# preethamam/AutomaticPanoramicImageStitching-AutoPanoStitch-MATLAB

Hardware: NVIDIA B200
Metric: descriptor_pairs_per_sec (higher is better)
Workload: dtype f16

## Files before the change

### automaticpanoramicimagestitching-autopanostitch-matlab_b200/csrc/aps_knn_tc.cu

```cuda
#include "aps_tc_ptx.cuh"

#pragma nv_diag_suppress 128

namespace {
using namespace aps_tc;

constexpr int TM = 128;
constexpr int RB = 2;
constexpr int TN = 128;
constexpr int NUM_B_STAGES = 4;
constexpr int NUM_ACC_SLOTS = 2 * RB;
constexpr int NUM_CS_STAGES = 8;
constexpr int KC = 8;
constexpr int CSPLIT = 1;
constexpr int MAX_SEG = 4 / CSPLIT;
constexpr int NUM_EPI_WARPS = 4 * RB * CSPLIT;
constexpr int FIRST_EPI_WARP = 1 + RB;
constexpr int NUM_THREADS = 32 * (FIRST_EPI_WARP + NUM_EPI_WARPS);
static_assert(NUM_ACC_SLOTS * TN == 512, "TMEM budget");

struct Barriers {
  uint64_t b_full[NUM_B_STAGES], b_empty[NUM_B_STAGES];
  uint64_t a_full, a_empty;
  uint64_t acc_full[NUM_ACC_SLOTS], acc_empty[NUM_ACC_SLOTS];
  uint64_t cs_full[NUM_CS_STAGES], cs_empty[NUM_CS_STAGES];
  uint32_t tmem_base;
  uint32_t pad;
};

__device__ __forceinline__ float4 lds_f32x4(uint32_t a) {
  float4 v;
  asm volatile("ld.shared.v4.f32 {%0, %1, %2, %3}, [%4];" : "=f"(v.x), "=f"(v.y), "=f"(v.z), "=f"(v.w) : "r"(a));
  return v;
}
__device__ __forceinline__ uint32_t lds_u32(uint32_t a) { uint32_t v; asm volatile("ld.shared.u32 %0, [%1];" : "=r"(v) : "r"(a)); return v; }
__device__ __forceinline__ void sts_u32(uint32_t a, uint32_t v) { asm volatile("st.shared.u32 [%0], %1;" ::"r"(a), "r"(v) : "memory"); }
constexpr uint32_t SLOT_STRIDE = TM * 4;

struct KParams {
  int64_t q0, q1, t0, t1;
  int dp;
  int nslot;
  int units_full;
  int tail_units;
  int tail_seg;
  int64_t tile_lo;
  int64_t tile_hi;
  int tiles_per_seg;
  int tail_balanced;
  int grid;
  const float* colscale;
// ... 69 lines not shown
__device__ __forceinline__ void top2_of_32(float (&v)[32]) {
#pragma unroll
  for (int i = 0; i < 32; i += 2) {
    const float a = v[i], b = v[i + 1];
    v[i] = fmaxf(a, b);
    v[i + 1] = fminf(a, b);
  }
#pragma unroll
  for (int st = 2; st < 32; st *= 2)
#pragma unroll
    for (int i = 0; i < 32; i += 2 * st) top2_merge(v[i], v[i + 1], v[i + st], v[i + st + 1]);
}
__device__ __forceinline__ void insert3(float x, uint32_t px, float& l1, float& l2, float& l3, uint32_t& p1, uint32_t& p2,
                                        uint32_t& p3) {
  const bool c1 = x > l1, c2 = x > l2, c3 = x > l3;
  l3 = c2 ? l2 : (c3 ? x : l3);
  p3 = c2 ? p2 : (c3 ? px : p3);
  l2 = c1 ? l1 : (c2 ? x : l2);
  p2 = c1 ? p1 : (c2 ? px : p2);
  l1 = c1 ? x : l1;
  p1 = c1 ? px : p1;
}
constexpr uint32_t kKeyFloorBits = 0xff7fff80u;
constexpr int threads_for(int cs) { return 32 * (1 + RB + 4 * RB * cs); }

template <bool BIAS, bool DUMP, bool PRE, int KCT, int CS = CSPLIT>
__global__ void __launch_bounds__(threads_for(CS), 1)
k_knn_tc(const __grid_constant__ CUtensorMap map_q, const __grid_constant__ CUtensorMap map_t, const KParams Pin) {
  if (Pin.variant_flag && ((*Pin.variant_flag != 0) != (Pin.variant_want != 0))) return;
  extern __shared__ __align__(1024) uint8_t smem_raw[];
  uint8_t* smem = (uint8_t*)(((uintptr_t)smem_raw + 1023) & ~(uintptr_t)1023);
  const int a_bytes = TM * Pin.dp * 2, b_bytes = TN * Pin.dp * 2;
  uint8_t* smem_a = smem;
  uint8_t* smem_b = smem_a + RB * a_bytes;
  float* smem_cs = (float*)(smem_b + NUM_B_STAGES * b_bytes);
  uint32_t* smem_topi = (uint32_t*)(smem_cs + NUM_CS_STAGES * 2 * TN);
  Barriers* bars = (Barriers*)(smem_topi + RB * CS * KC * TM);

  const int warp = threadIdx.x >> 5, lane = threadIdx.x & 31;
  const int ksl = Pin.dp / KSLAB;
  const int kst = Pin.dp / 16;
  KParams P = Pin;
  if (P.nrows_dev) {
    const int64_t n = *P.nrows_dev;
    P.q1 = P.q0 + n;
    P.units_full = 0;
    P.tail_units = (int)((n + RB * TM - 1) / (RB * TM));
  }
  const int64_t num_units = P.unit_table ? P.n_table_units
                            : (P.tail_balanced ? (int64_t)P.units_full + (int64_t)P.tail_balanced * P.grid
                                               : (int64_t)P.units_full + (int64_t)P.tail_units * P.tail_seg);

  if (threadIdx.x == 0) {
    for (int i = 0; i < NUM_B_STAGES; ++i) { mbar_init(&bars->b_full[i], 1); mbar_init(&bars->b_empty[i], RB); }
    mbar_init(&bars->a_full, 1);
    mbar_init(&bars->a_empty, RB);
    for (int i = 0; i < NUM_ACC_SLOTS; ++i) { mbar_init(&bars->acc_full[i], 1); mbar_init(&bars->acc_empty[i], 4 * CS); }
    for (int i = 0; i < NUM_CS_STAGES; ++i) { mbar_init(&bars->cs_full[i], 1); mbar_init(&bars->cs_empty[i], (4 * RB * CS)); }
    asm volatile("fence.mbarrier_init.release.cluster;" ::: "memory");
  }
  if (warp == 1) {
    asm volatile("tcgen05.alloc.cta_group::1.sync.aligned.shared::cta.b32 [%0], %1;" ::"r"(smem_u32(&bars->tmem_base)), "r"(512) : "memory");
    asm volatile("tcgen05.relinquish_alloc_permit.cta_group::1.sync.aligned;" ::: "memory");
  }
  tc_fence_before();
  __syncthreads();
  tc_fence_after();
  const uint32_t tmem_base = bars->tmem_base;

  if (warp == 0) {
    if (elect_one()) {
      uint32_t bs = 0, bph = 0, aph = 0, cs = 0, cph = 0;
      for (int64_t u = blockIdx.x; u < num_units; u += gridDim.x) {
        const Unit x = get_unit(P, u);
        if (x.tl >= x.th) continue;
        mbar_wait_backoff(&bars->a_empty, aph ^ 1);
        mbar_arrive_expect_tx(&bars->a_full, (uint32_t)(RB * a_bytes));
        for (int r = 0; r < RB; ++r)
          for (int s = 0; s < ksl; ++s)
            tma_load_2d(smem_a + r * a_bytes + s * (TM * 128), &map_q, s * KSLAB,
                        (int)(x.qrow0 + r * TM), &bars->a_full);
        aph ^= 1;
        for (int64_t t = x.tl; t < x.th; ++t) {
          mbar_wait_backoff(&bars->cs_empty[cs], cph ^ 1);
          mbar_arrive_expect_tx(&bars->cs_full[cs], (BIAS ? 2u : 1u) * TN * (uint32_t)sizeof(float));
          bulk_load_1d(smem_cs + cs * 2 * TN, P.colscale + t * TN, TN * (uint32_t)sizeof(float), &bars->cs_full[cs]);
          if (BIAS)
            bulk_load_1d(smem_cs + cs * 2 * TN + TN, P.colbias + t * TN, TN * (uint32_t)sizeof(float), &bars->cs_full[cs]);
          if (++cs == NUM_CS_STAGES) { cs = 0; cph ^= 1; }
          mbar_wait_backoff(&bars->b_empty[bs], bph ^ 1);
          mbar_arrive_expect_tx(&bars->b_full[bs], (uint32_t)b_bytes);
          for (int s = 0; s < ksl; ++s)
            tma_load_2d(smem_b + bs * b_bytes + s * (TN * 128), &map_t, s * KSLAB, (int)(t * TN), &bars->b_full[bs]);
          if (++bs == NUM_B_STAGES) { bs = 0; bph ^= 1; }
        }
      }
    }
  } else if (warp <= RB) {
    if (elect_one()) {
      const int r = warp - 1;
      const uint32_t idesc = P.idesc;
      const uint32_t a_addr = smem_u32(smem_a + r * a_bytes);
      uint32_t bs = 0, bph = 0, aph = 0, tcount = 0;
      for (int64_t u = blockIdx.x; u < num_units; u += gridDim.x) {
        const Unit x = get_unit(P, u);
        if (x.tl >= x.th) continue;
        mbar_wait(&bars->a_full, aph);
        aph ^= 1;
        for (int64_t t = x.tl; t < x.th; ++t, ++tcount) {
          const uint32_t slot = (tcount & 1) * RB + r, acph = (tcount >> 1) & 1;
          mbar_wait(&bars->acc_empty[slot], acph ^ 1);
          mbar_wait(&bars->b_full[bs], bph);
          tc_fence_after();
          const uint32_t b_addr = smem_u32(smem_b + bs * b_bytes);
          const uint32_t d_tmem = tmem_base + slot * TN;
          for (int k = 0; k < kst; ++k) {
            const int slab = k >> 2, kin = k & 3;
            const uint64_t adesc = make_kmajor_sw128_desc(a_addr + slab * (TM * 128) + kin * 32);
            const uint64_t bdesc = make_kmajor_sw128_desc(b_addr + slab * (TN * 128) + kin * 32);
            umma_bf16(d_tmem, adesc, bdesc, idesc, k > 0 ? 1u : 0u);
          }
          tc_commit(&bars->acc_full[slot]);
          tc_commit(&bars->b_empty[bs]);
          if (++bs == NUM_B_STAGES) { bs = 0; bph ^= 1; }
        }
        tc_commit(&bars->a_empty);
      }
    }
  } else {
    const int quad = warp & 3;
    const int egrp = (warp - FIRST_EPI_WARP) >> 2;
    const int grp = egrp / CS;
    const int ch = egrp % CS;
    constexpr int CG = TN / CS;
    const int row_in_tile = quad * 32 + lane;
    const uint32_t si = smem_u32(smem_topi + (egrp * KC) * TM + row_in_tile);
    uint32_t tcount = 0;
    for (int64_t u = blockIdx.x; u < num_units; u += gridDim.x) {
      const Unit x = get_unit(P, u);
      if (x.skip) continue;
      const int64_t qrow = x.qrow0 + grp * TM + row_in_tile;
      if constexpr (KCT == 3) {
        float l1 = __uint_as_float(kKeyFloorBits), l2 = l1, l3 = l1;
        uint32_t p1 = 0xffffffffu, p2 = 0xffffffffu, p3 = 0xffffffffu;
        for (int64_t t = x.tl; t < x.th; ++t, ++tcount) {
          const uint32_t slot = (tcount & 1) * RB + grp, acph = (tcount >> 1) & 1;
          const uint32_t cs = tcount % NUM_CS_STAGES, cph = (tcount / NUM_CS_STAGES) & 1;
          mbar_wait(&bars->acc_full[slot], acph);
          mbar_wait(&bars->cs_full[cs], cph);
          tc_fence_after();
          const uint32_t cscale = smem_u32(smem_cs + cs * 2 * TN + ch * CG);
          const int64_t col0 = t * TN + ch * CG;
          const bool partial = (col0 < x.t0) || (col0 + CG > x.t1);
          const uint32_t taddr = tmem_base + ((uint32_t)(quad * 32) << 16) + slot * TN + ch * CG;
          float m1 = __uint_as_float(kKeyFloorBits), m2 = m1;
#pragma unroll 1
          for (int c = 0; c < CG / 32; ++c) {
            float cur[32];
            tmem_ld32(taddr + c * 32, cur);
            tmem_wait_ld(cur);
#pragma unroll
            for (int g = 0; g < 4; ++g) {
              const float4 s0 = lds_f32x4(cscale + (c * 32 + 8 * g) * 4);
              const float4 s1 = lds_f32x4(cscale + (c * 32 + 8 * g + 4) * 4);
              if (BIAS) {
                const float4 b0 = lds_f32x4(cscale + (TN + c * 32 + 8 * g) * 4);
                const float4 b1 = lds_f32x4(cscale + (TN + c * 32 + 8 * g + 4) * 4);
                cur[8 * g + 0] = fmaf(cur[8 * g + 0], s0.x, b0.x); cur[8 * g + 1] = fmaf(cur[8 * g + 1], s0.y, b0.y);
                cur[8 * g + 2] = fmaf(cur[8 * g + 2], s0.z, b0.z); cur[8 * g + 3] = fmaf(cur[8 * g + 3], s0.w, b0.w);
                cur[8 * g + 4] = fmaf(cur[8 * g + 4], s1.x, b1.x); cur[8 * g + 5] = fmaf(cur[8 * g + 5], s1.y, b1.y);
                cur[8 * g + 6] = fmaf(cur[8 * g + 6], s1.z, b1.z); cur[8 * g + 7] = fmaf(cur[8 * g + 7], s1.w, b1.w);
              } else {
                cur[8 * g + 0] *= s0.x; cur[8 * g + 1] *= s0.y; cur[8 * g + 2] *= s0.z; cur[8 * g + 3] *= s0.w;
                cur[8 * g + 4] *= s1.x; cur[8 * g + 5] *= s1.y; cur[8 * g + 6] *= s1.z; cur[8 * g + 7] *= s1.w;
              }
            }
            const uint32_t cbase = (uint32_t)(ch * CG + c * 32);
#pragma unroll
            for (int j = 0; j < 32; ++j)
              cur[j] = __uint_as_float((__float_as_uint(cur[j]) & ~127u) | (cbase + (uint32_t)j));
            if (partial) {
              const int lo = (int)max(x.t0 - col0, (int64_t)0) - c * 32, hi = (int)min(x.t1 - col0, (int64_t)CG) - c * 32;
#pragma unroll
              for (int j = 0; j < 32; ++j)
                if (j < lo || j >= hi) cur[j] = __uint_as_float(kKeyFloorBits | (cbase + (uint32_t)j));
            }
            top2_of_32(cur);
            top2_merge(m1, m2, cur[0], cur[1]);
          }
          tc_fence_before();
          __syncwarp();
          if (lane == 0) {
            mbar_arrive(&bars->acc_empty[slot]);
            mbar_arrive(&bars->cs_empty[cs]);
          }
          const uint32_t base = (uint32_t)(t * TN);
          insert3(m1, base + (__float_as_uint(m1) & 127u), l1, l2, l3, p1, p2, p3);
          insert3(m2, base + (__float_as_uint(m2) & 127u), l1, l2, l3, p1, p2, p3);
        }
        if (qrow < x.qend) {
          const int64_t o = (x.out_row + grp * TM + row_in_tile) * P.cand_stride + ch * 3;
          const float floor_v = -1.0e38f;
          P.cand_idx[o + 0] = l1 > floor_v ? p1 : 0xffffffffu; P.cand_score[o + 0] = l1 > floor_v ? l1 : -CUDART_INF_F;
          P.cand_idx[o + 1] = l2 > floor_v ? p2 : 0xffffffffu; P.cand_score[o + 1] = l2 > floor_v ? l2 : -CUDART_INF_F;
          P.cand_idx[o + 2] = l3 > floor_v ? p3 : 0xffffffffu; P.cand_score[o + 2] = l3 > floor_v ? l3 : -CUDART_INF_F;
        }
        continue;
      }
      float bv[KCT];
#pragma unroll
      for (int i = 0; i < KCT; ++i) {
        bv[i] = __uint_as_float(0xff7ffff8u | (uint32_t)i);
        sts_u32(si + i * SLOT_STRIDE, 0xffffffffu);
      }
      float theta = bv[KCT - 1];
      int minpos = KCT - 1;
      float4 tb_next = (PRE && x.tl < x.th) ? __ldg(P.tile_bounds + x.tl) : make_float4(0.f, 0.f, 0.f, 0.f);
      for (int64_t t = x.tl; t < x.th; ++t, ++tcount) {
        const uint32_t slot = (tcount & 1) * RB + grp, acph = (tcount >> 1) & 1;
        const uint32_t cs = tcount % NUM_CS_STAGES, cph = (tcount / NUM_CS_STAGES) & 1;
        mbar_wait(&bars->acc_full[slot], acph);
        mbar_wait(&bars->cs_full[cs], cph);
        tc_fence_after();
        const uint32_t cscale = smem_u32(smem_cs + cs * 2 * TN + ch * CG);
        const int64_t col0 = t * TN + ch * CG;
        const bool partial = (col0 < x.t0) || (col0 + CG > x.t1);
        const uint32_t taddr = tmem_base + ((uint32_t)(quad * 32) << 16) + slot * TN + ch * CG;
        const float4 tb = tb_next;
        if (PRE && t + 1 < x.th) tb_next = __ldg(P.tile_bounds + t + 1);
        auto pre_threshold = [&](float th) {
          const float num = th - tb.z - 1.0e-6f * (fabsf(th) + fabsf(tb.z));
          return num * (num >= 0.f ? tb.x : tb.y);
        };
        float thr_pre = PRE ? pre_threshold(theta) : 0.f;
        float va[32], vb[32];
        bool slot_released = false;
        if constexpr (PRE && CS == 1 && !DUMP) {
#ifndef APS_TC_NOEPI
          float rm[16];
          tmem_ld32(taddr, va);
          tmem_wait_ld(va);
#pragma unroll
          for (int c = 0; c < 4; ++c) {
            float(&cur)[32] = (c & 1) ? vb : va;
            float(&nxt)[32] = (c & 1) ? va : vb;
            if (c + 1 < 4) tmem_ld32(taddr + (c + 1) * 32, nxt);
#pragma unroll
            for (int g = 0; g < 4; ++g) {
              float m = fmaxf(fmaxf(cur[8 * g], cur[8 * g + 1]), cur[8 * g + 2]);
              m = fmaxf(fmaxf(m, cur[8 * g + 3]), cur[8 * g + 4]);
              m = fmaxf(fmaxf(m, cur[8 * g + 5]), cur[8 * g + 6]);
              rm[4 * c + g] = fmaxf(m, cur[8 * g + 7]);
            }
            if (c + 1 < 4) tmem_wait_ld(nxt);
          }
          float tmax = fmaxf(fmaxf(rm[0], rm[1]), rm[2]);
#pragma unroll
          for (int g = 3; g < 15; g += 2) tmax = fmaxf(fmaxf(tmax, rm[g]), rm[g + 1]);
          tmax = fmaxf(tmax, rm[15]);
          if (__any_sync(0xffffffffu, partial || tmax > thr_pre)) {
            uint32_t pend = 0;
#pragma unroll
            for (int g = 0; g < 16; ++g) pend |= (rm[g] > thr_pre) ? (1u << g) : 0u;
            if (partial) pend = 0xffffu;
            uint32_t uni = __reduce_or_sync(0xffffffffu, pend);
            auto search_group = [&](float(&v)[8], const int g) {
              const float4 s0 = lds_f32x4(cscale + (8 * g) * 4);
              const float4 s1 = lds_f32x4(cscale + (8 * g + 4) * 4);
              if (BIAS) {
                const float4 b0 = lds_f32x4(cscale + (TN + 8 * g) * 4);
                const float4 b1 = lds_f32x4(cscale + (TN + 8 * g + 4) * 4);
                v[0] = fmaf(v[0], s0.x, b0.x); v[1] = fmaf(v[1], s0.y, b0.y);
                v[2] = fmaf(v[2], s0.z, b0.z); v[3] = fmaf(v[3], s0.w, b0.w);
                v[4] = fmaf(v[4], s1.x, b1.x); v[5] = fmaf(v[5], s1.y, b1.y);
                v[6] = fmaf(v[6], s1.z, b1.z); v[7] = fmaf(v[7], s1.w, b1.w);
              } else {
                v[0] *= s0.x; v[1] *= s0.y; v[2] *= s0.z; v[3] *= s0.w;
                v[4] *= s1.x; v[5] *= s1.y; v[6] *= s1.z; v[7] *= s1.w;
              }
              if (partial) {
#pragma unroll
                for (int j = 0; j < 8; ++j) {
                  const int64_t col = col0 + 8 * g + j;
                  if (col < x.t0 || col >= x.t1) v[j] = -CUDART_INF_F;
                }
              }
              float gm = fmaxf(fmaxf(v[0], v[1]), v[2]);
              gm = fmaxf(fmaxf(gm, v[3]), v[4]);
              gm = fmaxf(fmaxf(gm, v[5]), v[6]);
              gm = fmaxf(gm, v[7]);
              while (gm > theta) {
                int js = 7;
#pragma unroll
                for (int j = 6; j >= 0; --j) js = (v[j] == gm) ? j : js;
                sts_u32(si + minpos * SLOT_STRIDE, (uint32_t)(col0 + 8 * g + js));
                const float key = __uint_as_float((__float_as_uint(gm) & ~7u) | (uint32_t)minpos);
#pragma unroll
                for (int i = 0; i < KCT; ++i) bv[i] = (i == minpos) ? key : bv[i];
                if constexpr (KCT == 8) {
                  float m01 = fminf(fminf(bv[0], bv[1]), bv[2]);
                  float m23 = fminf(fminf(bv[3], bv[4]), bv[5]);
                  theta = fminf(fminf(m01, m23), fminf(bv[6], bv[7]));
                } else if constexpr (KCT == 6) {
                  theta = fminf(fminf(fminf(bv[0], bv[1]), bv[2]), fminf(fminf(bv[3], bv[4]), bv[5]));
                } else {
                  theta = fminf(fminf(bv[0], bv[1]), fminf(bv[2], bv[3]));
                }
                minpos = (int)(__float_as_uint(theta) & 7u);
#pragma unroll
                for (int j = 0; j < 8; ++j) v[j] = (j == js) ? -CUDART_INF_F : v[j];
                gm = fmaxf(fmaxf(v[0], v[1]), v[2]);
                gm = fmaxf(fmaxf(gm, v[3]), v[4]);
                gm = fmaxf(fmaxf(gm, v[5]), v[6]);
                gm = fmaxf(gm, v[7]);
              }
            };
            while (uni) {
              int gq[4];
#pragma unroll
              for (int q = 0; q < 4; ++q) {
                gq[q] = uni ? __ffs((int)uni) - 1 : 31;
                uni &= uni - 1;
              }
              float vs[32];
              __syncwarp();
#pragma unroll
              for (int q = 0; q < 4; ++q) tmem_ld8(taddr + 8 * (gq[q] & 15), *reinterpret_cast<float(*)[8]>(vs + 8 * q));
              tmem_wait_ld(vs);
              if (uni == 0u) {
                tc_fence_before();
                __syncwarp();
                if (lane == 0) mbar_arrive(&bars->acc_empty[slot]);
                slot_released = true;
              }
#pragma unroll
              for (int q = 0; q < 4; ++q)
                if ((pend >> gq[q]) & 1u) search_group(*reinterpret_cast<float(*)[8]>(vs + 8 * q), gq[q]);
            }
          }
#endif
        } else {
        if (CS == 1) {
          tmem_ld32(taddr, va);
          tmem_wait_ld(va);
        }
#pragma unroll 1
        for (int c2 = 0; c2 < CG / 64 + (CG % 64 ? 1 : 0); ++c2) {
#pragma unroll
          for (int h = 0; h < (CG >= 64 ? 2 : 1); ++h) {
            const int c = 2 * c2 + h;
            float(&cur)[32] = (CS == 1 && h) ? vb : va;
            float(&nxt)[32] = (CS == 1 && h) ? va : vb;
            if (CS == 1) {
              if (c + 1 < CG / 32) tmem_ld32(taddr + (c + 1) * 32, nxt);
            } else {
              tmem_ld32(taddr + c * 32, cur);
              tmem_wait_ld(cur);
            }
            float rm[4] = {0.f, 0.f, 0.f, 0.f};
            if (PRE) {
// ... 56 lines not shown
                      theta = fminf(fminf(bv[0], bv[1]), fminf(bv[2], bv[3]));
                    } else {
                      theta = fminf(fminf(bv[0], bv[1]), bv[2]);
                    }
                    minpos = (int)(__float_as_uint(theta) & 7u);
#pragma unroll
                    for (int j = 0; j < 8; ++j) cur[8 * g + j] = (j == js) ? -CUDART_INF_F : cur[8 * g + j];
                    gm = fmaxf(fmaxf(cur[8 * g], cur[8 * g + 1]), cur[8 * g + 2]);
                    gm = fmaxf(fmaxf(gm, cur[8 * g + 3]), cur[8 * g + 4]);
                    gm = fmaxf(fmaxf(gm, cur[8 * g + 5]), cur[8 * g + 6]);
                    gm = fmaxf(gm, cur[8 * g + 7]);
                  }
                }
              }
              if (PRE && inserted) thr_pre = pre_threshold(theta);
            }
            if (CS == 1 && c + 1 < CG / 32) tmem_wait_ld(nxt);
          }
        }
        }
        tc_fence_before();
        __syncwarp();
        if (lane == 0) {
          if (!slot_released) mbar_arrive(&bars->acc_empty[slot]);
          mbar_arrive(&bars->cs_empty[cs]);
        }
      }
      if (qrow < x.qend) {
        const int cstr = P.cand_stride;
        const int64_t o = ((x.out_row + grp * TM + row_in_tile) * P.nslot + x.seg * CS + ch) * cstr;
#pragma unroll
        for (int i = 0; i < KCT; ++i) {
          P.cand_idx[o + i] = lds_u32(si + i * SLOT_STRIDE);
          P.cand_score[o + i] = bv[i];
        }
        for (int i = KCT; i < cstr; ++i) {
          P.cand_idx[o + i] = 0xffffffffu;
          P.cand_score[o + i] = -CUDART_INF_F;
        }
        if (ch == 0)
          for (int sl = x.clear_from - x.seg * CS; sl < P.nslot - x.seg * CS; ++sl)
            for (int i = 0; i < cstr; ++i) {
              P.cand_idx[o + sl * cstr + i] = 0xffffffffu;
              P.cand_score[o + sl * cstr + i] = -CUDART_INF_F;
            }
      }
    }
  }
  tc_fence_before();
  __syncthreads();
  if (warp == 1) {
    tc_fence_after();
    asm volatile("tcgen05.dealloc.cta_group::1.sync.aligned.b32 %0, %1;" ::"r"(tmem_base), "r"(512) : "memory");
  }
}

}

int aps_k_knn_tc_supported(int Dp) { return Dp == 64 || Dp == 128; }
int aps_k_knn_tc_tile_rows() { return TN; }
int aps_k_knn_tc_tile_mode_stride() { return 2 * 3; }
int aps_k_knn_tc_tile_mode_segment() { return TN / 2; }

struct TcSchedule {
  int units_full, tail_units, tail_seg, nslot, tiles_per_seg, tail_balanced;
  int64_t tile_lo, tile_hi;
};
static TcSchedule make_schedule(int sm_count, int64_t nq, int64_t t0, int64_t t1, bool all_segmented = false) {
  TcSchedule sc;
  sc.tail_balanced = 0;
  if (all_segmented) {
    sc.tile_lo = t0 / TN;
    sc.tile_hi = aps_ceil_div(t1, TN);
    const int64_t tiles = sc.tile_hi - sc.tile_lo;
    sc.units_full = 0;
    sc.tail_units = (int)aps_ceil_div(nq, (int64_t)RB * TM);
    sc.tail_seg = (int)(tiles < MAX_SEG ? (tiles < 1 ? 1 : tiles) : MAX_SEG);
    sc.nslot = sc.tail_seg * CSPLIT;
    sc.tiles_per_seg = (int)aps_ceil_div(tiles, sc.tail_seg);
// ... 90 lines not shown
  P.cand_idx = p.cand_idx;
  P.cand_score = p.cand_score;
  P.dump = p.dump;
  P.unit_table = nullptr;
  P.n_table_units = 0;
  P.cand_stride = KC;
  P.variant_flag = nullptr;
  P.variant_want = 0;
  P.idesc = p.operand_fp16 ? make_idesc_f16_f32acc(TM, TN) : make_idesc_bf16(TM, TN);
  P.nrows_dev = p.nrows_dev;
  if (p.nrows_dev) {
    P.units_full = 0;
    P.tail_units = (int)aps_ceil_div(p.q1 - p.q0, (int64_t)RB * TM);
    P.tail_seg = sc.tail_seg;
    P.tiles_per_seg = sc.tiles_per_seg;
  }
  const size_t smem = 1024 + (size_t)RB * TM * p.Dp * 2 + (size_t)NUM_B_STAGES * TN * p.Dp * 2 +
                      (size_t)NUM_CS_STAGES * 2 * TN * sizeof(float) + (size_t)RB * CSPLIT * KC * TM * 4 + sizeof(Barriers);
  const int64_t units = sc.tail_balanced ? (int64_t)sc.units_full + (int64_t)sc.tail_balanced * sm_count
                                         : (int64_t)sc.units_full + (int64_t)sc.tail_units * sc.tail_seg;
  const unsigned grid = (unsigned)(units < sm_count ? units : sm_count);
  if (ev0) APS_CUDA(cudaEventRecord(ev0, s));
  auto launch = [&](auto kern) -> int {
    APS_CUDA(cudaFuncSetAttribute(kern, cudaFuncAttributeMaxDynamicSharedMemorySize, (int)smem));
    kern<<<grid, NUM_THREADS, smem, s>>>(map_q, map_t, P);
    return APS_OK;
  };
  const int64_t sweep = (sc.tile_hi - sc.tile_lo) / ((sc.units_full && !p.nrows_dev) ? 1 : (sc.tail_seg > 0 ? sc.tail_seg : 1));
  const bool pre = sweep >= 96 && p.tile_bounds != nullptr;
  if (p.dump)
    APS_TRY(p.bias ? launch(k_knn_tc<true, true, false, KC>) : launch(k_knn_tc<false, true, false, KC>));
  else if (p.exact_flag && !p.nrows_dev) {
    P.variant_flag = p.exact_flag;
    P.variant_want = 1;
    if (pre)
      APS_TRY(p.bias ? launch(k_knn_tc<true, false, true, 6>) : launch(k_knn_tc<false, false, true, 6>));
    else
      APS_TRY(p.bias ? launch(k_knn_tc<true, false, false, 6>) : launch(k_knn_tc<false, false, false, 6>));
    APS_LAUNCHED();
    P.variant_want = 0;
    if (pre)
      APS_TRY(p.bias ? launch(k_knn_tc<true, false, true, KC>) : launch(k_knn_tc<false, false, true, KC>));
    else
      APS_TRY(p.bias ? launch(k_knn_tc<true, false, false, KC>) : launch(k_knn_tc<false, false, false, KC>));
  } else if (pre)
    APS_TRY(p.bias ? launch(k_knn_tc<true, false, true, KC>) : launch(k_knn_tc<false, false, true, KC>));
  else
// ... 32 lines not shown
  CUtensorMap map_q, map_t;
  const CUtensorMapDataType dt = p.operand_fp16 ? CU_TENSOR_MAP_DATA_TYPE_FLOAT16 : CU_TENSOR_MAP_DATA_TYPE_BFLOAT16;
  APS_TRY(make_map(&map_q, p.Qb, p.Fq_total, p.Dp, TM, dt));
  APS_TRY(make_map(&map_t, p.Tb, p.Ft_total, p.Dp, TN, dt));
  KParams P;
  memset(&P, 0, sizeof P);
  P.idesc = p.operand_fp16 ? make_idesc_f16_f32acc(TM, TN) : make_idesc_bf16(TM, TN);
  P.nrows_dev = nullptr;
  P.dp = p.Dp;
  P.nslot = 1;
  P.colscale = p.colscale;
  P.colbias = p.colbias;
  P.tile_bounds = p.tile_bounds;
  P.cand_idx = p.cand_idx;
  P.cand_score = p.cand_score;
  P.dump = nullptr;
  P.unit_table = d_units;
  P.n_table_units = n_units;
  P.cand_stride = p.kcand;
  const int cs_groups = p.kcand == 3 ? 2 : CSPLIT;
  const size_t smem = 1024 + (size_t)RB * TM * p.Dp * 2 + (size_t)NUM_B_STAGES * TN * p.Dp * 2 +
                      (size_t)NUM_CS_STAGES * 2 * TN * sizeof(float) + (size_t)RB * cs_groups * KC * TM * 4 + sizeof(Barriers);
  const unsigned grid = (unsigned)(n_units < sm_count ? n_units : sm_count);
  int threads = NUM_THREADS;
  auto launch = [&](auto kern) -> int {
    APS_CUDA(cudaFuncSetAttribute(kern, cudaFuncAttributeMaxDynamicSharedMemorySize, (int)smem));
    kern<<<grid, threads, smem, s>>>(map_q, map_t, P);
    return APS_OK;
  };
  if (p.kcand == 3) {
    threads = threads_for(2);
    P.cand_stride = aps_k_knn_tc_tile_mode_stride();
    APS_TRY(p.bias ? launch(k_knn_tc<true, false, false, 3, 2>) : launch(k_knn_tc<false, false, false, 3, 2>));
  } else if (p.kcand == 4)
    APS_TRY(p.bias ? launch(k_knn_tc<true, false, false, 4>) : launch(k_knn_tc<false, false, false, 4>));
  else if (p.kcand == KC)
    APS_TRY(p.bias ? launch(k_knn_tc<true, false, false, KC>) : launch(k_knn_tc<false, false, false, KC>));
  else {
    aps_set_error(APS_ERR_ARGS, "", "kcand must be 3, 4 or %d", KC);
    return APS_ERR_ARGS;
  }
  APS_LAUNCHED();
  return APS_OK;
}
```

### automaticpanoramicimagestitching-autopanostitch-matlab_b200/csrc/aps_tc_ptx.cuh

```cuda
#pragma once
#include <cstdio>
#include <cuda.h>
#include <math_constants.h>

#include "aps_common.cuh"

namespace aps_tc {

constexpr int KSLAB = 64;

static __device__ __forceinline__ uint32_t smem_u32(const void* p) { return (uint32_t)__cvta_generic_to_shared(p); }

static __device__ __forceinline__ bool elect_one() {
  uint32_t pred;
  asm volatile(
      "{\n\t.reg .pred p;\n\t"
      "elect.sync _|p, 0xffffffff;\n\t"
      "selp.u32 %0, 1, 0, p;\n\t}"
      : "=r"(pred));
  return pred != 0;
}
static __device__ __forceinline__ void mbar_init(uint64_t* bar, uint32_t count) {
  asm volatile("mbarrier.init.shared::cta.b64 [%0], %1;" ::"r"(smem_u32(bar)), "r"(count) : "memory");
}
static __device__ __forceinline__ void mbar_arrive(uint64_t* bar) {
  asm volatile("mbarrier.arrive.shared::cta.b64 _, [%0];" ::"r"(smem_u32(bar)) : "memory");
}
static __device__ __forceinline__ void mbar_arrive_expect_tx(uint64_t* bar, uint32_t bytes) {
  asm volatile("mbarrier.arrive.expect_tx.shared::cta.b64 _, [%0], %1;" ::"r"(smem_u32(bar)), "r"(bytes) : "memory");
}
constexpr uint32_t kSuspendHintNs = 20000;
static __device__ __forceinline__ void mbar_wait(uint64_t* bar, uint32_t parity) {
  const uint32_t addr = smem_u32(bar);
  uint32_t done;
#ifdef APS_TC_WATCHDOG
  uint32_t spins = 0;
#endif
  do {
    asm volatile(
        "{\n\t.reg .pred p;\n\t"
        "mbarrier.try_wait.parity.shared::cta.b64 p, [%1], %2, %3;\n\t"
        "selp.u32 %0, 1, 0, p;\n\t}"
        : "=r"(done)
        : "r"(addr), "r"(parity), "r"(kSuspendHintNs)
        : "memory");
#ifdef APS_TC_WATCHDOG
    if (!done && ++spins > (1u << 16)) {
      printf("mbar watchdog: block %d thread %d barrier smem+0x%x parity %u\n", (int)blockIdx.x, (int)threadIdx.x, addr, parity);
      __trap();
    }
#endif
  } while (!done);
}
static __device__ __forceinline__ void mbar_wait_backoff(uint64_t* bar, uint32_t parity) {
  const uint32_t addr = smem_u32(bar);
  uint32_t done;
  for (;;) {
    asm volatile(
        "{\n\t.reg .pred p;\n\t"
        "mbarrier.try_wait.parity.shared::cta.b64 p, [%1], %2, %3;\n\t"
        "selp.u32 %0, 1, 0, p;\n\t}"
        : "=r"(done)
        : "r"(addr), "r"(parity), "r"(kSuspendHintNs)
        : "memory");
    if (done) break;
    __nanosleep(40);
  }
}
static __device__ __forceinline__ void tma_load_2d(void* dst, const CUtensorMap* map, int c0, int c1, uint64_t* bar) {
  asm volatile(
      "cp.async.bulk.tensor.2d.shared::cluster.global.tile.mbarrier::complete_tx::bytes [%0], [%1, {%2, %3}], [%4];"
      ::"r"(smem_u32(dst)), "l"(map), "r"(c0), "r"(c1), "r"(smem_u32(bar))
      : "memory");
}
static __device__ __forceinline__ void bulk_load_1d(void* dst, const void* src, uint32_t bytes, uint64_t* bar) {
  asm volatile("cp.async.bulk.shared::cluster.global.mbarrier::complete_tx::bytes [%0], [%1], %2, [%3];"
               ::"r"(smem_u32(dst)), "l"(src), "r"(bytes), "r"(smem_u32(bar))
               : "memory");
}
static __device__ __forceinline__ void tc_fence_before() { asm volatile("tcgen05.fence::before_thread_sync;" ::: "memory"); }
static __device__ __forceinline__ void tc_fence_after() { asm volatile("tcgen05.fence::after_thread_sync;" ::: "memory"); }
static __device__ __forceinline__ void tc_commit(uint64_t* bar) {
  asm volatile("tcgen05.commit.cta_group::1.mbarrier::arrive::one.shared::cluster.b64 [%0];" ::"r"(smem_u32(bar))
               : "memory");
}
static __device__ __forceinline__ void umma_bf16(uint32_t tmem_d, uint64_t adesc, uint64_t bdesc, uint32_t idesc,
                                          uint32_t accumulate) {
  asm volatile(
      "{\n\t.reg .pred p;\n\t"
      "setp.ne.b32 p, %4, 0;\n\t"
      "tcgen05.mma.cta_group::1.kind::f16 [%0], %1, %2, %3, p;\n\t}"
      ::"r"(tmem_d), "l"(adesc), "l"(bdesc), "r"(idesc), "r"(accumulate)
      : "memory");
}
static __device__ __forceinline__ void tmem_ld32(uint32_t taddr, float (&v)[32]) {
  uint32_t* r = reinterpret_cast<uint32_t*>(v);
  asm volatile(
      "tcgen05.ld.sync.aligned.32x32b.x32.b32 {%0, %1, %2, %3, %4, %5, %6, %7, %8, %9, %10, %11, %12, %13, %14, %15, "
      "%16, %17, %18, %19, %20, %21, %22, %23, %24, %25, %26, %27, %28, %29, %30, %31}, [%32];"
      : "=r"(r[0]), "=r"(r[1]), "=r"(r[2]), "=r"(r[3]), "=r"(r[4]), "=r"(r[5]), "=r"(r[6]), "=r"(r[7]), "=r"(r[8]),
        "=r"(r[9]), "=r"(r[10]), "=r"(r[11]), "=r"(r[12]), "=r"(r[13]), "=r"(r[14]), "=r"(r[15]), "=r"(r[16]),
        "=r"(r[17]), "=r"(r[18]), "=r"(r[19]), "=r"(r[20]), "=r"(r[21]), "=r"(r[22]), "=r"(r[23]), "=r"(r[24]),
        "=r"(r[25]), "=r"(r[26]), "=r"(r[27]), "=r"(r[28]), "=r"(r[29]), "=r"(r[30]), "=r"(r[31])
      : "r"(taddr)
      : "memory");
}
static __device__ __forceinline__ void tmem_ld8(uint32_t taddr, float (&v)[8]) {
  uint32_t* r = reinterpret_cast<uint32_t*>(v);
// ... 86 lines not shown
```

Before: 4873 billion.

## Rebalance registers across warp roles and streamline barrier and scale handling in kNN kernel

Pads the producer and MMA-issuer warps out to a full warpgroup so setmaxnreg can be used: the control warps shrink their register allocation and the epilogue warps grow theirs. This aims to cut register pressure and spills in the top-k epilogue. Barrier and TMEM addresses are precomputed as 32-bit offsets with parity toggles, replacing per-tile div/mod arithmetic and 64-bit column math. The PRE path skips the scale ring, and the search groups now read colscale/colbias through __ldg rather than shared memory. A host check fails the launch if the compiled register count does not match the assumed split, and an A/B benchmark script is added.

```diff
diff --git a/automaticpanoramicimagestitching-autopanostitch-matlab_b200/csrc/aps_knn_tc.cu b/automaticpanoramicimagestitching-autopanostitch-matlab_b200/csrc/aps_knn_tc.cu
--- a/automaticpanoramicimagestitching-autopanostitch-matlab_b200/csrc/aps_knn_tc.cu
+++ b/automaticpanoramicimagestitching-autopanostitch-matlab_b200/csrc/aps_knn_tc.cu
@@ -15,7 +15,8 @@
 constexpr int CSPLIT = 1;
 constexpr int MAX_SEG = 4 / CSPLIT;
 constexpr int NUM_EPI_WARPS = 4 * RB * CSPLIT;
-constexpr int FIRST_EPI_WARP = 1 + RB;
+constexpr int FIRST_EPI_WARP = 4;
+static_assert(1 + RB <= FIRST_EPI_WARP, "producer and issuers fit in warpgroup 0");
 constexpr int NUM_THREADS = 32 * (FIRST_EPI_WARP + NUM_EPI_WARPS);
 static_assert(NUM_ACC_SLOTS * TN == 512, "TMEM budget");
 
@@ -27,6 +28,8 @@
   uint32_t tmem_base;
   uint32_t pad;
 };
+constexpr uint32_t kAccEmptyOff = offsetof(Barriers, acc_empty) - offsetof(Barriers, acc_full);
+constexpr uint32_t kCsEmptyOff = offsetof(Barriers, cs_empty) - offsetof(Barriers, cs_full);
 
 __device__ __forceinline__ float4 lds_f32x4(uint32_t a) {
   float4 v;
@@ -142,11 +145,18 @@
   p1 = c1 ? px : p1;
 }
 constexpr uint32_t kKeyFloorBits = 0xff7fff80u;
-constexpr int threads_for(int cs) { return 32 * (1 + RB + 4 * RB * cs); }
+__host__ __device__ constexpr int threads_for(int cs) { return 32 * (FIRST_EPI_WARP + 4 * RB * cs); }
+__host__ __device__ constexpr int ctl_regs(int cs) { return cs == 1 ? 48 : 64; }
+__host__ __device__ constexpr int launch_regs(int cs) { return (65536 / threads_for(cs)) & ~7; }
+__host__ __device__ constexpr int epi_regs(int cs) {
+  return ((launch_regs(cs) * threads_for(cs) - 128 * ctl_regs(cs)) / (threads_for(cs) - 128)) & ~7;
+}
+static_assert(epi_regs(1) == 224 && epi_regs(2) == 104, "register split");
 
 template <bool BIAS, bool DUMP, bool PRE, int KCT, int CS = CSPLIT>
 __global__ void __launch_bounds__(threads_for(CS), 1)
 k_knn_tc(const __grid_constant__ CUtensorMap map_q, const __grid_constant__ CUtensorMap map_t, const KParams Pin) {
+  static_assert(!PRE || (CS == 1 && !DUMP), "PRE has no (scale, bias) ring");
   if (Pin.variant_flag && ((*Pin.variant_flag != 0) != (Pin.variant_want != 0))) return;
   extern __shared__ __align__(1024) uint8_t smem_raw[];
   uint8_t* smem = (uint8_t*)(((uintptr_t)smem_raw + 1023) & ~(uintptr_t)1023);
@@ -188,66 +198,76 @@
   tc_fence_after();
   const uint32_t tmem_base = bars->tmem_base;
 
-  if (warp == 0) {
-    if (elect_one()) {
-      uint32_t bs = 0, bph = 0, aph = 0, cs = 0, cph = 0;
-      for (int64_t u = blockIdx.x; u < num_units; u += gridDim.x) {
-        const Unit x = get_unit(P, u);
-        if (x.tl >= x.th) continue;
-        mbar_wait_backoff(&bars->a_empty, aph ^ 1);
-        mbar_arrive_expect_tx(&bars->a_full, (uint32_t)(RB * a_bytes));
-        for (int r = 0; r < RB; ++r)
-          for (int s = 0; s < ksl; ++s)
-            tma_load_2d(smem_a + r * a_bytes + s * (TM * 128), &map_q, s * KSLAB,
-                        (int)(x.qrow0 + r * TM), &bars->a_full);
-        aph ^= 1;
-        for (int64_t t = x.tl; t < x.th; ++t) {
-          mbar_wait_backoff(&bars->cs_empty[cs], cph ^ 1);
-          mbar_arrive_expect_tx(&bars->cs_full[cs], (BIAS ? 2u : 1u) * TN * (uint32_t)sizeof(float));
-          bulk_load_1d(smem_cs + cs * 2 * TN, P.colscale + t * TN, TN * (uint32_t)sizeof(float), &bars->cs_full[cs]);
-          if (BIAS)
-            bulk_load_1d(smem_cs + cs * 2 * TN + TN, P.colbias + t * TN, TN * (uint32_t)sizeof(float), &bars->cs_full[cs]);
-          if (++cs == NUM_CS_STAGES) { cs = 0; cph ^= 1; }
-          mbar_wait_backoff(&bars->b_empty[bs], bph ^ 1);
-          mbar_arrive_expect_tx(&bars->b_full[bs], (uint32_t)b_bytes);
-          for (int s = 0; s < ksl; ++s)
-            tma_load_2d(smem_b + bs * b_bytes + s * (TN * 128), &map_t, s * KSLAB, (int)(t * TN), &bars->b_full[bs]);
-          if (++bs == NUM_B_STAGES) { bs = 0; bph ^= 1; }
+  if (warp < FIRST_EPI_WARP) {
+    asm volatile("setmaxnreg.dec.sync.aligned.u32 %0;" ::"n"(ctl_regs(CS)));
+    if (warp == 0) {
+      if (elect_one()) {
+        uint32_t bs = 0, bph = 0, aph = 0, cs = 0, cph = 0;
+        for (int64_t u = blockIdx.x; u < num_units; u += gridDim.x) {
+          const Unit x = get_unit(P, u);
+          if (x.tl >= x.th) continue;
+          mbar_wait_backoff(&bars->a_empty, aph ^ 1);
+          mbar_arrive_expect_tx(&bars->a_full, (uint32_t)(RB * a_bytes));
+          for (int r = 0; r < RB; ++r)
+            for (int s = 0; s < ksl; ++s)
+              tma_load_2d(smem_a + r * a_bytes + s * (TM * 128), &map_q, s * KSLAB,
+                          (int)(x.qrow0 + r * TM), &bars->a_full);
+          aph ^= 1;
+          for (int64_t t = x.tl; t < x.th; ++t) {
+            if constexpr (!PRE) {
+              mbar_wait_backoff(&bars->cs_empty[cs], cph ^ 1);
+              mbar_arrive_expect_tx(&bars->cs_full[cs], (BIAS ? 2u : 1u) * TN * (uint32_t)sizeof(float));
+              bulk_load_1d(smem_cs + cs * 2 * TN, P.colscale + t * TN, TN * (uint32_t)sizeof(float), &bars->cs_full[cs]);
+              if (BIAS)
+                bulk_load_1d(smem_cs + cs * 2 * TN + TN, P.colbias + t * TN, TN * (uint32_t)sizeof(float), &bars->cs_full[cs]);
+              if (++cs == NUM_CS_STAGES) { cs = 0; cph ^= 1; }
+            }
+            mbar_wait_backoff(&bars->b_empty[bs], bph ^ 1);
+            mbar_arrive_expect_tx(&bars->b_full[bs], (uint32_t)b_bytes);
+            for (int s = 0; s < ksl; ++s)
+              tma_load_2d(smem_b + bs * b_bytes + s * (TN * 128), &map_t, s * KSLAB, (int)(t * TN), &bars->b_full[bs]);
+            if (++bs == NUM_B_STAGES) { bs = 0; bph ^= 1; }
+          }
         }
       }
-    }
-  } else if (warp <= RB) {
-    if (elect_one()) {
-      const int r = warp - 1;
-      const uint32_t idesc = P.idesc;
-      const uint32_t a_addr = smem_u32(smem_a + r * a_bytes);
-      uint32_t bs = 0, bph = 0, aph = 0, tcount = 0;
-      for (int64_t u = blockIdx.x; u < num_units; u += gridDim.x) {
-        const Unit x = get_unit(P, u);
-        if (x.tl >= x.th) continue;
-        mbar_wait(&bars->a_full, aph);
-        aph ^= 1;
-        for (int64_t t = x.tl; t < x.th; ++t, ++tcount) {
-          const uint32_t slot = (tcount & 1) * RB + r, acph = (tcount >> 1) & 1;
-          mbar_wait(&bars->acc_empty[slot], acph ^ 1);
-          mbar_wait(&bars->b_full[bs], bph);
-          tc_fence_after();
-          const uint32_t b_addr = smem_u32(smem_b + bs * b_bytes);
-          const uint32_t d_tmem = tmem_base + slot * TN;
-          for (int k = 0; k < kst; ++k) {
-            const int slab = k >> 2, kin = k & 3;
-            const uint64_t adesc = make_kmajor_sw128_desc(a_addr + slab * (TM * 128) + kin * 32);
-            const uint64_t bdesc = make_kmajor_sw128_desc(b_addr + slab * (TN * 128) + kin * 32);
-            umma_bf16(d_tmem, adesc, bdesc, idesc, k > 0 ? 1u : 0u);
+    } else if (warp <= RB) {
+      if (elect_one()) {
+        const int r = warp - 1;
+        const uint32_t idesc = P.idesc;
+        const uint32_t a_addr = smem_u32(smem_a + r * a_bytes);
+        const uint32_t b_addr0 = smem_u32(smem_b);
+        const uint32_t b_full0 = smem_u32(&bars->b_full[0]), b_empty0 = smem_u32(&bars->b_empty[0]);
+        const uint32_t acc_bar = smem_u32(&bars->acc_full[r]);
+        uint32_t bs = 0, bph = 0, aph = 0, par = 0, acph = 0;
+        for (int64_t u = blockIdx.x; u < num_units; u += gridDim.x) {
+          const Unit x = get_unit(P, u);
+          if (x.tl >= x.th) continue;
+          mbar_wait(&bars->a_full, aph);
+          aph ^= 1;
+          for (uint32_t i = 0, n = (uint32_t)(x.th - x.tl); i < n; ++i) {
+            mbar_wait(acc_bar + kAccEmptyOff + par * (RB * 8), acph ^ 1);
+            mbar_wait(b_full0 + bs * 8, bph);
+            tc_fence_after();
+            const uint32_t b_addr = b_addr0 + bs * b_bytes;
+            const uint32_t d_tmem = tmem_base + (par * RB + r) * TN;
+            for (int k = 0; k < kst; ++k) {
+              const int slab = k >> 2, kin = k & 3;
+              const uint64_t adesc = make_kmajor_sw128_desc(a_addr + slab * (TM * 128) + kin * 32);
+              const uint64_t bdesc = make_kmajor_sw128_desc(b_addr + slab * (TN * 128) + kin * 32);
+              umma_bf16(d_tmem, adesc, bdesc, idesc, k > 0 ? 1u : 0u);
+            }
+            tc_commit(acc_bar + par * (RB * 8));
+            tc_commit(b_empty0 + bs * 8);
+            if (++bs == NUM_B_STAGES) { bs = 0; bph ^= 1; }
+            par ^= 1;
+            acph ^= par ^ 1;
           }
-          tc_commit(&bars->acc_full[slot]);
-          tc_commit(&bars->b_empty[bs]);
-          if (++bs == NUM_B_STAGES) { bs = 0; bph ^= 1; }
-        }
-        tc_commit(&bars->a_empty);
+          tc_commit(&bars->a_empty);
+        }
       }
     }
   } else {
+    asm volatile("setmaxnreg.inc.sync.aligned.u32 %0;" ::"n"(epi_regs(CS)));
     const int quad = warp & 3;
     const int egrp = (warp - FIRST_EPI_WARP) >> 2;
     const int grp = egrp / CS;
@@ -255,24 +275,31 @@
     constexpr int CG = TN / CS;
     const int row_in_tile = quad * 32 + lane;
     const uint32_t si = smem_u32(smem_topi + (egrp * KC) * TM + row_in_tile);
-    uint32_t tcount = 0;
+    const uint32_t acc_bar = smem_u32(&bars->acc_full[grp]), cs_bar = smem_u32(&bars->cs_full[0]);
+    const uint32_t cs_smem0 = smem_u32(smem_cs + ch * CG);
+    const uint32_t tmem_row = tmem_base + ((uint32_t)(quad * 32) << 16) + grp * TN + ch * CG;
+    uint32_t par = 0, acph = 0, cs = 0, cph = 0;
+    auto next_tile = [&]() {
+      par ^= 1;
+      acph ^= par ^ 1;
+      if (!PRE && ++cs == NUM_CS_STAGES) { cs = 0; cph ^= 1; }
+    };
     for (int64_t u = blockIdx.x; u < num_units; u += gridDim.x) {
       const Unit x = get_unit(P, u);
       if (x.skip) continue;
       const int64_t qrow = x.qrow0 + grp * TM + row_in_tile;
+      const uint32_t nt = x.th > x.tl ? (uint32_t)(x.th - x.tl) : 0u, ct0 = (uint32_t)x.t0, ct1 = (uint32_t)x.t1;
       if constexpr (KCT == 3) {
         float l1 = __uint_as_float(kKeyFloorBits), l2 = l1, l3 = l1;
         uint32_t p1 = 0xffffffffu, p2 = 0xffffffffu, p3 = 0xffffffffu;
-        for (int64_t t = x.tl; t < x.th; ++t, ++tcount) {
-          const uint32_t slot = (tcount & 1) * RB + grp, acph = (tcount >> 1) & 1;
-          const uint32_t cs = tcount % NUM_CS_STAGES, cph = (tcount / NUM_CS_STAGES) & 1;
-          mbar_wait(&bars->acc_full[slot], acph);
-          mbar_wait(&bars->cs_full[cs], cph);
+        uint32_t col0 = (uint32_t)(x.tl * TN) + ch * CG;
+        for (uint32_t i = 0; i < nt; ++i, col0 += TN, next_tile()) {
+          mbar_wait(acc_bar + par * (RB * 8), acph);
+          mbar_wait(cs_bar + cs * 8, cph);
           tc_fence_after();
-          const uint32_t cscale = smem_u32(smem_cs + cs * 2 * TN + ch * CG);
-          const int64_t col0 = t * TN + ch * CG;
-          const bool partial = (col0 < x.t0) || (col0 + CG > x.t1);
-          const uint32_t taddr = tmem_base + ((uint32_t)(quad * 32) << 16) + slot * TN + ch * CG;
+          const uint32_t cscale = cs_smem0 + cs * (2 * TN * 4);
+          const bool partial = (col0 < ct0) || (col0 + CG > ct1);
+          const uint32_t taddr = tmem_row + par * (RB * TN);
           float m1 = __uint_as_float(kKeyFloorBits), m2 = m1;
 #pragma unroll 1
           for (int c = 0; c < CG / 32; ++c) {
@@ -300,7 +327,7 @@
             for (int j = 0; j < 32; ++j)
               cur[j] = __uint_as_float((__float_as_uint(cur[j]) & ~127u) | (cbase + (uint32_t)j));
             if (partial) {
-              const int lo = (int)max(x.t0 - col0, (int64_t)0) - c * 32, hi = (int)min(x.t1 - col0, (int64_t)CG) - c * 32;
+              const int lo = max((int)(ct0 - col0), 0) - c * 32, hi = min((int)(ct1 - col0), CG) - c * 32;
 #pragma unroll
               for (int j = 0; j < 32; ++j)
                 if (j < lo || j >= hi) cur[j] = __uint_as_float(kKeyFloorBits | (cbase + (uint32_t)j));
@@ -311,10 +338,10 @@
           tc_fence_before();
           __syncwarp();
           if (lane == 0) {
-            mbar_arrive(&bars->acc_empty[slot]);
-            mbar_arrive(&bars->cs_empty[cs]);
+            mbar_arrive(acc_bar + kAccEmptyOff + par * (RB * 8));
+            mbar_arrive(cs_bar + kCsEmptyOff + cs * 8);
           }
-          const uint32_t base = (uint32_t)(t * TN);
+          const uint32_t base = col0 - ch * CG;
           insert3(m1, base + (__float_as_uint(m1) & 127u), l1, l2, l3, p1, p2, p3);
           insert3(m2, base + (__float_as_uint(m2) & 127u), l1, l2, l3, p1, p2, p3);
         }
@@ -335,19 +362,19 @@
       }
       float theta = bv[KCT - 1];
       int minpos = KCT - 1;
-      float4 tb_next = (PRE && x.tl < x.th) ? __ldg(P.tile_bounds + x.tl) : make_float4(0.f, 0.f, 0.f, 0.f);
-      for (int64_t t = x.tl; t < x.th; ++t, ++tcount) {
-        const uint32_t slot = (tcount & 1) * RB + grp, acph = (tcount >> 1) & 1;
-        const uint32_t cs = tcount % NUM_CS_STAGES, cph = (tcount / NUM_CS_STAGES) & 1;
-        mbar_wait(&bars->acc_full[slot], acph);
-        mbar_wait(&bars->cs_full[cs], cph);
+      const float4* tbp = P.tile_bounds + x.tl;
+      float4 tb_next = (PRE && nt > 0) ? __ldg(tbp) : make_float4(0.f, 0.f, 0.f, 0.f);
+      uint32_t col0 = (uint32_t)(x.tl * TN) + ch * CG;
+      for (uint32_t i = 0; i < nt; ++i, col0 += TN, next_tile()) {
+        const uint32_t acc_off = par * (RB * 8);
+        mbar_wait(acc_bar + acc_off, acph);
+        if (!PRE) mbar_wait(cs_bar + cs * 8, cph);
         tc_fence_after();
-        const uint32_t cscale = smem_u32(smem_cs + cs * 2 * TN + ch * CG);
-        const int64_t col0 = t * TN + ch * CG;
-        const bool partial = (col0 < x.t0) || (col0 + CG > x.t1);
-        const uint32_t taddr = tmem_base + ((uint32_t)(quad * 32) << 16) + slot * TN + ch * CG;
+        const uint32_t cscale = cs_smem0 + cs * (2 * TN * 4);
+        const bool partial = (col0 < ct0) || (col0 + CG > ct1);
+        const uint32_t taddr = tmem_row + par * (RB * TN);
         const float4 tb = tb_next;
-        if (PRE && t + 1 < x.th) tb_next = __ldg(P.tile_bounds + t + 1);
+        if (PRE && i + 1 < nt) tb_next = __ldg(tbp + i + 1);
         auto pre_threshold = [&](float th) {
           const float num = th - tb.z - 1.0e-6f * (fabsf(th) + fabsf(tb.z));
           return num * (num >= 0.f ? tb.x : tb.y);
@@ -384,12 +411,10 @@
             for (int g = 0; g < 16; ++g) pend |= (rm[g] > thr_pre) ? (1u << g) : 0u;
             if (partial) pend = 0xffffu;
             uint32_t uni = __reduce_or_sync(0xffffffffu, pend);
-            auto search_group = [&](float(&v)[8], const int g) {
-              const float4 s0 = lds_f32x4(cscale + (8 * g) * 4);
-              const float4 s1 = lds_f32x4(cscale + (8 * g + 4) * 4);
+            auto search_group = [&](float(&v)[8], const int g, const float4 (&s)[2], const float4 (&b)[2]) {
+              const float4 s0 = s[0], s1 = s[1];
               if (BIAS) {
-                const float4 b0 = lds_f32x4(cscale + (TN + 8 * g) * 4);
-                const float4 b1 = lds_f32x4(cscale + (TN + 8 * g + 4) * 4);
+                const float4 b0 = b[0], b1 = b[1];
                 v[0] = fmaf(v[0], s0.x, b0.x); v[1] = fmaf(v[1], s0.y, b0.y);
                 v[2] = fmaf(v[2], s0.z, b0.z); v[3] = fmaf(v[3], s0.w, b0.w);
                 v[4] = fmaf(v[4], s1.x, b1.x); v[5] = fmaf(v[5], s1.y, b1.y);
@@ -401,8 +426,8 @@
               if (partial) {
 #pragma unroll
                 for (int j = 0; j < 8; ++j) {
-                  const int64_t col = col0 + 8 * g + j;
-                  if (col < x.t0 || col >= x.t1) v[j] = -CUDART_INF_F;
+                  const uint32_t col = col0 + 8 * g + j;
+                  if (col < ct0 || col >= ct1) v[j] = -CUDART_INF_F;
                 }
               }
               float gm = fmaxf(fmaxf(v[0], v[1]), v[2]);
@@ -413,10 +438,10 @@
                 int js = 7;
 #pragma unroll
                 for (int j = 6; j >= 0; --j) js = (v[j] == gm) ? j : js;
-                sts_u32(si + minpos * SLOT_STRIDE, (uint32_t)(col0 + 8 * g + js));
+                sts_u32(si + minpos * SLOT_STRIDE, col0 + 8 * g + js);
                 const float key = __uint_as_float((__float_as_uint(gm) & ~7u) | (uint32_t)minpos);
 #pragma unroll
-                for (int i = 0; i < KCT; ++i) bv[i] = (i == minpos) ? key : bv[i];
+                for (int k = 0; k < KCT; ++k) bv[k] = (k == minpos) ? key : bv[k];
                 if constexpr (KCT == 8) {
                   float m01 = fminf(fminf(bv[0], bv[1]), bv[2]);
                   float m23 = fminf(fminf(bv[3], bv[4]), bv[5]);
@@ -442,6 +467,18 @@
                 gq[q] = uni ? __ffs((int)uni) - 1 : 31;
                 uni &= uni - 1;
               }
+              float4 gs[4][2], gb[4][2];
+#pragma unroll
+              for (int q = 0; q < 4; ++q) {
+                const float4* s4 = reinterpret_cast<const float4*>(P.colscale + col0 + 8 * (gq[q] & 15));
+                gs[q][0] = __ldg(s4);
+                gs[q][1] = __ldg(s4 + 1);
+                if (BIAS) {
+                  const float4* b4 = reinterpret_cast<const float4*>(P.colbias + col0 + 8 * (gq[q] & 15));
+                  gb[q][0] = __ldg(b4);
+                  gb[q][1] = __ldg(b4 + 1);
+                }
+              }
               float vs[32];
               __syncwarp();
 #pragma unroll
@@ -450,12 +487,12 @@
               if (uni == 0u) {
                 tc_fence_before();
                 __syncwarp();
-                if (lane == 0) mbar_arrive(&bars->acc_empty[slot]);
+                if (lane == 0) mbar_arrive(acc_bar + kAccEmptyOff + acc_off);
                 slot_released = true;
               }
 #pragma unroll
               for (int q = 0; q < 4; ++q)
-                if ((pend >> gq[q]) & 1u) search_group(*reinterpret_cast<float(*)[8]>(vs + 8 * q), gq[q]);
+                if ((pend >> gq[q]) & 1u) search_group(*reinterpret_cast<float(*)[8]>(vs + 8 * q), gq[q], gs[q], gb[q]);
             }
           }
 #endif
@@ -558,8 +595,8 @@
         tc_fence_before();
         __syncwarp();
         if (lane == 0) {
-          if (!slot_released) mbar_arrive(&bars->acc_empty[slot]);
-          mbar_arrive(&bars->cs_empty[cs]);
+          if (!slot_released) mbar_arrive(acc_bar + kAccEmptyOff + acc_off);
+          if (!PRE) mbar_arrive(cs_bar + kCsEmptyOff + cs * 8);
         }
       }
       if (qrow < x.qend) {
@@ -591,6 +628,19 @@
   }
 }
 
+}
+
+template <typename Kern>
+static int prepare_launch(Kern kern, int cs, size_t smem) {
+  APS_CUDA(cudaFuncSetAttribute(kern, cudaFuncAttributeMaxDynamicSharedMemorySize, (int)smem));
+  cudaFuncAttributes fa;
+  APS_CUDA(cudaFuncGetAttributes(&fa, kern));
+  if (fa.numRegs != launch_regs(cs)) {
+    aps_set_error(APS_ERR_CUDA, "", "k_knn_tc allocates %d registers per thread, the register split assumes %d",
+                  fa.numRegs, launch_regs(cs));
+    return APS_ERR_CUDA;
+  }
+  return APS_OK;
 }
 
 int aps_k_knn_tc_supported(int Dp) { return Dp == 64 || Dp == 128; }
@@ -727,7 +777,7 @@
   const unsigned grid = (unsigned)(units < sm_count ? units : sm_count);
   if (ev0) APS_CUDA(cudaEventRecord(ev0, s));
   auto launch = [&](auto kern) -> int {
-    APS_CUDA(cudaFuncSetAttribute(kern, cudaFuncAttributeMaxDynamicSharedMemorySize, (int)smem));
+    APS_TRY(prepare_launch(kern, CSPLIT, smem));
     kern<<<grid, NUM_THREADS, smem, s>>>(map_q, map_t, P);
     return APS_OK;
   };
@@ -806,14 +856,13 @@
   const size_t smem = 1024 + (size_t)RB * TM * p.Dp * 2 + (size_t)NUM_B_STAGES * TN * p.Dp * 2 +
                       (size_t)NUM_CS_STAGES * 2 * TN * sizeof(float) + (size_t)RB * cs_groups * KC * TM * 4 + sizeof(Barriers);
   const unsigned grid = (unsigned)(n_units < sm_count ? n_units : sm_count);
-  int threads = NUM_THREADS;
+  const int threads = threads_for(cs_groups);
   auto launch = [&](auto kern) -> int {
-    APS_CUDA(cudaFuncSetAttribute(kern, cudaFuncAttributeMaxDynamicSharedMemorySize, (int)smem));
+    APS_TRY(prepare_launch(kern, cs_groups, smem));
     kern<<<grid, threads, smem, s>>>(map_q, map_t, P);
     return APS_OK;
   };
   if (p.kcand == 3) {
-    threads = threads_for(2);
     P.cand_stride = aps_k_knn_tc_tile_mode_stride();
     APS_TRY(p.bias ? launch(k_knn_tc<true, false, false, 3, 2>) : launch(k_knn_tc<false, false, false, 3, 2>));
   } else if (p.kcand == 4)
diff --git a/automaticpanoramicimagestitching-autopanostitch-matlab_b200/csrc/aps_tc_ptx.cuh b/automaticpanoramicimagestitching-autopanostitch-matlab_b200/csrc/aps_tc_ptx.cuh
--- a/automaticpanoramicimagestitching-autopanostitch-matlab_b200/csrc/aps_tc_ptx.cuh
+++ b/automaticpanoramicimagestitching-autopanostitch-matlab_b200/csrc/aps_tc_ptx.cuh
@@ -23,15 +23,15 @@
 static __device__ __forceinline__ void mbar_init(uint64_t* bar, uint32_t count) {
   asm volatile("mbarrier.init.shared::cta.b64 [%0], %1;" ::"r"(smem_u32(bar)), "r"(count) : "memory");
 }
-static __device__ __forceinline__ void mbar_arrive(uint64_t* bar) {
-  asm volatile("mbarrier.arrive.shared::cta.b64 _, [%0];" ::"r"(smem_u32(bar)) : "memory");
+static __device__ __forceinline__ void mbar_arrive(uint32_t bar) {
+  asm volatile("mbarrier.arrive.shared::cta.b64 _, [%0];" ::"r"(bar) : "memory");
 }
+static __device__ __forceinline__ void mbar_arrive(uint64_t* bar) { mbar_arrive(smem_u32(bar)); }
 static __device__ __forceinline__ void mbar_arrive_expect_tx(uint64_t* bar, uint32_t bytes) {
   asm volatile("mbarrier.arrive.expect_tx.shared::cta.b64 _, [%0], %1;" ::"r"(smem_u32(bar)), "r"(bytes) : "memory");
 }
 constexpr uint32_t kSuspendHintNs = 20000;
-static __device__ __forceinline__ void mbar_wait(uint64_t* bar, uint32_t parity) {
-  const uint32_t addr = smem_u32(bar);
+static __device__ __forceinline__ void mbar_wait(uint32_t addr, uint32_t parity) {
   uint32_t done;
 #ifdef APS_TC_WATCHDOG
   uint32_t spins = 0;
@@ -52,6 +52,7 @@
 #endif
   } while (!done);
 }
+static __device__ __forceinline__ void mbar_wait(uint64_t* bar, uint32_t parity) { mbar_wait(smem_u32(bar), parity); }
 static __device__ __forceinline__ void mbar_wait_backoff(uint64_t* bar, uint32_t parity) {
   const uint32_t addr = smem_u32(bar);
   uint32_t done;
@@ -80,10 +81,10 @@
 }
 static __device__ __forceinline__ void tc_fence_before() { asm volatile("tcgen05.fence::before_thread_sync;" ::: "memory"); }
 static __device__ __forceinline__ void tc_fence_after() { asm volatile("tcgen05.fence::after_thread_sync;" ::: "memory"); }
-static __device__ __forceinline__ void tc_commit(uint64_t* bar) {
-  asm volatile("tcgen05.commit.cta_group::1.mbarrier::arrive::one.shared::cluster.b64 [%0];" ::"r"(smem_u32(bar))
-               : "memory");
+static __device__ __forceinline__ void tc_commit(uint32_t bar) {
+  asm volatile("tcgen05.commit.cta_group::1.mbarrier::arrive::one.shared::cluster.b64 [%0];" ::"r"(bar) : "memory");
 }
+static __device__ __forceinline__ void tc_commit(uint64_t* bar) { tc_commit(smem_u32(bar)); }
 static __device__ __forceinline__ void umma_bf16(uint32_t tmem_d, uint64_t adesc, uint64_t bdesc, uint32_t idesc,
                                           uint32_t accumulate) {
   asm volatile(
diff --git a/profiles/ab_bench.py b/profiles/ab_bench.py
--- /dev/null
+++ b/profiles/ab_bench.py
@@ -0,0 +1,74 @@
+from __future__ import annotations
+
+import argparse
+import filecmp
+import json
+import os
+import statistics
+import subprocess
+import sys
+
+
+def run_bench(tree, config, extra=()):
+    cmd = [sys.executable, os.path.join(tree, "bench.py"), "--config", config, "--no-cpu-baseline", "--no-extra", *extra]
+    r = subprocess.run(cmd, capture_output=True, text=True, timeout=900)
+    lines = [l for l in r.stdout.splitlines() if l.startswith("{")]
+    if r.returncode or not lines:
+        raise SystemExit(f"{' '.join(cmd)} failed ({r.returncode}):\n{r.stdout[-2000:]}\n{r.stderr[-2000:]}")
+    return json.loads(lines[-1])
+
+
+def card():
+    q = subprocess.run(["nvidia-smi", "--query-gpu=name,power.limit,clocks.max.sm", "--format=csv,noheader"],
+                       capture_output=True, text=True)
+    return q.stdout.strip().splitlines()[0] if q.returncode == 0 and q.stdout.strip() else "unknown"
+
+
+def compare_dumps(a, b):
+    names = sorted(set(os.listdir(a)) | set(os.listdir(b)))
+    bad = [n for n in names if not (os.path.exists(os.path.join(a, n)) and os.path.exists(os.path.join(b, n))
+                                    and filecmp.cmp(os.path.join(a, n), os.path.join(b, n), shallow=False))]
+    return names, bad
+
+
+def main():
+    ap = argparse.ArgumentParser()
+    ap.add_argument("--old", required=True)
+    ap.add_argument("--new", required=True)
+    ap.add_argument("--runs", type=int, default=5)
+    ap.add_argument("--configs", default="c2")
+    ap.add_argument("--dump", default="", help="configs whose --dump-outputs files are compared byte for byte")
+    ap.add_argument("--out", required=True)
+    a = ap.parse_args()
+    os.makedirs(a.out, exist_ok=True)
+    trees = {"old": os.path.abspath(a.old), "new": os.path.abspath(a.new)}
+    print("card (name, power limit, max SM clock):", card(), flush=True)
+    for c in filter(None, a.dump.split(",")):
+        dirs = {}
+        for b, t in trees.items():
+            dirs[b] = os.path.join(os.path.abspath(a.out), f"dump_{c}_{b}")
+            line = run_bench(t, c, ("--dump-outputs", dirs[b]))
+            print(f"dump {c} {b}: parity_check={line.get('parity_check')}", flush=True)
+        names, bad = compare_dumps(dirs["old"], dirs["new"])
+        print(f"dump {c}: {len(names)} files {names}, " + ("byte-identical" if not bad else f"DIFFER: {bad}"), flush=True)
+    for c in filter(None, a.configs.split(",")):
+        res = {"old": [], "new": []}
+        with open(os.path.join(a.out, f"ab_{c}.jsonl"), "w") as f:
+            for i in range(a.runs):
+                for b in (("old", "new") if i % 2 == 0 else ("new", "old")):
+                    line = run_bench(trees[b], c)
+                    res[b].append(line)
+                    f.write(json.dumps({"build": b, "run": i, **line}) + "\n")
+                    f.flush()
+                    print(f"{c} run {i} {b}: ms_per_step {line['ms_per_step']:.4f} kernel_ms "
+                          f"{line.get('roofline', {}).get('kernel_ms', float('nan')):.4f} clocks {line.get('clocks')}", flush=True)
+        for b in ("old", "new"):
+            ms = [l["ms_per_step"] for l in res[b]]
+            km = [l.get("roofline", {}).get("kernel_ms", float("nan")) for l in res[b]]
+            print(f"{c} {b}: ms_per_step median {statistics.median(ms):.4f} range {min(ms):.4f}-{max(ms):.4f} | "
+                  f"kernel_ms median {statistics.median(km):.4f} range {min(km):.4f}-{max(km):.4f} | n={len(ms)}",
+                  flush=True)
+
+
+if __name__ == "__main__":
+    main()
```

Result: faster. 5094 billion, median of 6 (+4.5%).
